# Audio-WestlakeU/FN-SSL

Hardware: AMD Instinct MI355X
Metric: TF-frames/sec DP-IPD forward, 4-mic 257-bin x 300-frame (higher is better)
Workload: dtype f32; 1 GPU; BASELINE configs[1]: FN-SSL (online) DP-IPD forward, waveform->STFT->features->3x(full-band BiLSTM + narrow-band LSTM)->head; 32 utterances/GPU x 4 mics ('MM' = 6 pairs) x 257 bins x 300 frames, fp32; frame = one STFT frame of one utterance; stream_chunk_frames=0, utterances_per_gpu=32, global_batch=32, mics=4, pairs_per_utterance=6, frames=300, bins=257, parallelism=dp1 (utterance shards, no collective), chunk_pairs=0

## Files before the change

fn-ssl_amd/csrc/lstm_f32c.h:

```cpp
#pragma once

#include "lstm_static.h"

namespace fnssl_lstm {

constexpr int kF32cWaves = 16;

struct F32ClusterParams {
  unsigned* tags;
  unsigned* status;
  int clusters_per_dir;
  int groups_per_cluster;
  unsigned spin_limit;
  int stall_member;
  int rotate;
  int prio_mode;
};

template <int HH, int NV0, int NS0, int MODE, bool ABLRT = false, int DRIFT = 2, int NW_ = kF32cWaves, int GS = 1>
__global__ void __launch_bounds__(NW_ * 64) lstm_f32c_kernel(const LstmParams p, const F32ClusterParams cp) {
  constexpr int H = HH, NS = H / 16, NW = NW_;
  constexpr int NWS = NW / GS;
  static_assert((GS == 1 || GS == 4) && NW % GS == 0 && (NWS & (NWS - 1)) == 0, "gate split: whole slots, a power of two of them");
  constexpr bool SUM = (MODE & kSum) != 0, SAVE = (MODE & kSave) != 0;
  constexpr bool CAT = (MODE & kHas2) != 0;
  constexpr int QPS = 1 + NV0 + NS0 + NS;
  constexpr int XD = NW_ > 12 ? 4 : 8;
  constexpr bool STRH = H == 256 && GS == 1 && NW_ > 8;
  static_assert((CAT ? NS0 == 1 : !(NV0 && NS0)) && (NV0 == 0 || NV0 % XD == 0) && (H == 128 || H == 256),
                "blocks of src0, or its remainder alone, or blocks of src0 + the remainder quad of src2");
  static_assert(H == 128 || NW_ <= 8 || STRH, "H = 256 with the row of h_{t-1} held: at most two waves per SIMD (register budget)");
  static_assert(!STRH || (NV0 >= XD && (NV0 + NS) % XD == 0), "streamed row: the ring depth divides the block count");
  static_assert(GS == 1 || (!SAVE && !ABLRT), "gate split: inference kernels only");
  extern __shared__ __attribute__((aligned(16))) char smem[];
  const int ABL = ABLRT ? p.ablate : 0;

  const int b = blockIdx.x;
  const int m = (b >> 3) % NS;
  const int cl = ((b >> 3) / NS) * 8 + (b & 7);
  if (cl >= cp.clusters_per_dir * p.ndir) return;
  const int dir = cl / cp.clusters_per_dir;
  const int ck = cl - dir * cp.clusters_per_dir;
  const int g0 = ck * cp.groups_per_cluster;
  const int g1 = g0 + cp.groups_per_cluster < p.ntasks ? g0 + cp.groups_per_cluster : p.ntasks;
  if (__hip_atomic_load(cp.status, __ATOMIC_RELAXED, __HIP_MEMORY_SCOPE_AGENT) != 0) return;
  if (cl == 0 && m == cp.stall_member) return;

  const int lane = threadIdx.x & 63;
  const int n = lane & 15, g = lane >> 4;
  const int w = __builtin_amdgcn_readfirstlane((int)(threadIdx.x >> 6));
  const int ws = GS == 1 ? w : (w >> 2);
  const int gate = GS == 1 ? 0 : (w & 3);
  const bool rev = dir == 1;
  const unsigned vlane = lane * 16;

  {
    const v4f* src = reinterpret_cast<const v4f*>(reinterpret_cast<const char*>(p.wpack[dir]) + (size_t)(m * QPS) * 4096);
    v4f* dst = reinterpret_cast<v4f*>(smem);
    for (int i = threadIdx.x; i < QPS * 4 * 64; i += NW * 64) dst[i] = src[i];
  }
  char* const xch = smem + QPS * 4096;
  unsigned* const xcnt = reinterpret_cast<unsigned*>(xch + NWS * 2 * 4 * 1024);
  if (GS > 1 && threadIdx.x < NWS) xcnt[threadIdx.x] = 0;
  __syncthreads();
  const char* const lds_rd = smem + lane * 16;
  auto rec = [&](int q, int j) { return *reinterpret_cast<const v4f*>(lds_rd + (q * 4 + j) * 1024); };
  auto rec1 = [&](int q, int j) { return *reinterpret_cast<const float*>(lds_rd + (q * 4 + j) * 1024 + 4 * gate); };

  const unsigned st0 = (unsigned)(p.src0.st * 4), sto = (unsigned)(p.out_st * 4), stk = SUM ? (unsigned)(p.skip.st * 4) : 0u;
  const unsigned st2 = CAT ? (unsigned)(p.src2.st * 4) : 0u;
  const unsigned cy = (unsigned)p.carry;
  unsigned* const tag_cl = cp.tags + (size_t)cl * cp.groups_per_cluster * NS;
  const v4f zero4 = v4f{0.f, 0.f, 0.f, 0.f};

  unsigned pub_val = 0;
  unsigned* pub_tag = nullptr;
  auto pub_flush = [&]() {
    if (pub_tag) {
      asm volatile("s_waitcnt vmcnt(0)" ::: "memory");
      if (lane == 0) __hip_atomic_store(pub_tag, pub_val, __ATOMIC_RELAXED, __HIP_MEMORY_SCOPE_AGENT);
      pub_tag = nullptr;
    }
  };

  struct Grp {
    unsigned vo0, voo, vok, voo2, vo2 = 0;
    bool valid;
    int task, step;
  };
  auto locate = [&](int task, int qo0, int qi0, Grp& gr, rsrc_t& rx0, rsrc_t& ro, rsrc_t& rsk, rsrc_t& ro2, rsrc_t& rx2) {
    const int q0 = task * 16;
    gr.valid = q0 + n < p.nseq;
    const int d = q0 + n < p.nseq ? n : p.nseq - 1 - q0;
    const bool crossed = qi0 + d >= p.q_inner;
    auto one = [&](const float* base, long long so, long long si, int extra, unsigned& voff) {
      const long long delta = (long long)d * si + (crossed ? so - (long long)p.q_inner * si : 0ll);
      voff = (unsigned)(delta * 4) + (unsigned)(extra * 4);
      return make_rsrc(base + ((long long)qo0 * so + (long long)qi0 * si));
    };
    rx0 = one(p.src0.p, p.src0.so, p.src0.si, (NS0 && !CAT) ? g : 4 * g, gr.vo0);
    if constexpr (CAT) rx2 = one(p.src2.p, p.src2.so, p.src2.si, g, gr.vo2);
    ro = one(p.out, p.out_so, p.out_si, dir * H + 4 * g, gr.voo);
    gr.vok = gr.voo2 = 0;
    rsk = SUM ? one(p.skip.p, p.skip.so, p.skip.si, dir * H + 4 * g, gr.vok) : rx0;
    ro2 = SUM ? one(p.out_sum, p.out_so, p.out_si, dir * H + 4 * g, gr.voo2) : ro;
  };
  auto tt_of = [&](int step) { return (unsigned)(rev ? p.nsteps - 1 - step : step); };
  auto rc_of = [&](int task) {
    return make_rsrc(cell_record<NS>(p.cscratch, p.ntasks, dir, task));
  };

  if (g0 + ws >= g1) return;
  unsigned long long clk0 = 0, rt0 = 0;
  if (ABLRT && (ABL & 512)) {
    clk0 = __builtin_amdgcn_s_memtime();
    rt0 = __builtin_amdgcn_s_memrealtime();
  }
  bool dead = false;
  auto bounded_wait = [&](auto ready, auto reload, int sleep, unsigned code) {
    for (unsigned spins = 0; !ready(); ++spins) {
      if (GS > 1) __builtin_amdgcn_s_sleep(1); else if (sleep == 8) __builtin_amdgcn_s_sleep(8); else __builtin_amdgcn_s_sleep(16);
      reload();
      const bool out = spins > cp.spin_limit;
      if (out || (spins & 63) == 63) {
        if (out) {
          if (lane == 0) __hip_atomic_store(cp.status, code | (unsigned)(cl & 0xffff), __ATOMIC_RELAXED, __HIP_MEMORY_SCOPE_AGENT);
          return false;
        }
        if (__hip_atomic_load(cp.status, __ATOMIC_RELAXED, __HIP_MEMORY_SCOPE_AGENT) != 0) return false;
      }
    }
    return true;
  };
  const int NGR = g1 - g0;
  const bool rot = cp.rotate && NGR >= 2 * NWS;
  const int FULL = rot ? (NGR / NWS) * NWS : NGR, LEFT = NGR - FULL;
  const bool single = GS == 1 && g0 + ws + NWS >= g1;
  Grp cur, nxt;
  rsrc_t rx0, ro, rsk, ro2, rx2, nrx0, nro, nrsk, nro2, nrx2;
  v4f xr[XD];
  float xs0 = 0.f;
  v4f cprev = zero4, skipv = zero4;
  unsigned tagv = 0, tagd = 0;
  auto request = [&](const Grp& gr, rsrc_t qx0, rsrc_t qsk, bool with_c, bool with_x = true) {
    const unsigned tt = tt_of(gr.step);
    if (!(ABL & 8)) {
      if constexpr (NV0 > 0) if (with_x) static_for<XD>([&](auto v) { xr[v.value] = bld4(qx0, gr.vo0, tt * st0 + 64 * v.value); });
      if constexpr (NS0 > 0 && !CAT) xs0 = bld1(qx0, gr.vo0, tt * st0);
    }
    if (SUM && !(ABL & 64)) skipv = bld4(qsk, gr.vok, tt * stk + 64 * m);
    if (gr.step > 0 || cy) {
      if (gr.step > 0 && !(ABL & 256))
        tagv = __hip_atomic_load(tag_cl + (size_t)(gr.task - g0) * NS + (lane & (NS - 1)), __ATOMIC_RELAXED, __HIP_MEMORY_SCOPE_AGENT);
      if (GS == 1 && with_c && !(ABL & 64)) cprev = bld4_l2(rc_of(gr.task), vlane, m * 1024);
    }
    if (DRIFT > 0 && !(ABL & 256) && gr.task - DRIFT * NWS >= g0)
      tagd = __hip_atomic_load(tag_cl + (size_t)(gr.task - DRIFT * NWS - g0) * NS + (lane & (NS - 1)), __ATOMIC_RELAXED, __HIP_MEMORY_SCOPE_AGENT);
  };
  cur.task = g0 + ws;
  cur.step = 0;
  unsigned iter = 0;
  const int qo_first = (cur.task * 16) / p.q_inner, qi_first = cur.task * 16 - qo_first * p.q_inner;
  int qo0 = qo_first, qi0 = qi_first;
  locate(cur.task, qo0, qi0, cur, rx0, ro, rsk, ro2, rx2);
  request(cur, rx0, rsk, true);
  if constexpr (CAT) xs0 = bld1(rx2, cur.vo2, tt_of(0) * st2);

  for (;;) {
    const int step = cur.step, task = cur.task;
    const unsigned tt = tt_of(step);
    const unsigned o0 = tt * st0, oo = (tt + cy) * sto;
    const unsigned op = (rev ? tt + 1 : tt - 1 + cy) * sto;
    const rsrc_t rc = rc_of(task);
    unsigned* const tag_g = tag_cl + (size_t)(task - g0) * NS;
    if (single && (step > 0 || cy) && !(ABL & 64)) cprev = bld4_l2(rc, vlane, m * 1024);
    const bool late_c = GS > 1 || task >= g0 + FULL;
    v4f cprev_cur = (step > 0 || cy) ? cprev : zero4;
    const v4f skip_cur = skipv;

    v4f hold[STRH ? 1 : NS];
    auto fetch_h = [&]() {
      if (DRIFT > 0 && !(ABL & 4) && !dead && task - DRIFT * NWS >= g0) {
        unsigned* const tag_d = tag_cl + (size_t)(task - DRIFT * NWS - g0) * NS;
        dead = !bounded_wait([&]() { return __builtin_amdgcn_ballot_w64(tagd < (unsigned)step + 1) == 0; },
                             [&]() { tagd = __hip_atomic_load(tag_d + (lane & (NS - 1)), __ATOMIC_RELAXED, __HIP_MEMORY_SCOPE_AGENT); }, 8, 0x40000u);
      }
      if ((step > 0 || cy) && !(ABL & 16)) {
        if (step > 0 && !(ABL & 4) && !dead)
          dead = !bounded_wait([&]() { return __builtin_amdgcn_ballot_w64(tagv < (unsigned)step) == 0; },
                               [&]() { tagv = __hip_atomic_load(tag_g + (lane & (NS - 1)), __ATOMIC_RELAXED, __HIP_MEMORY_SCOPE_AGENT); }, 16, 0x30000u);
        if (late_c && !(ABL & 64)) cprev_cur = bld4_l2(rc, vlane, m * 1024);
        if constexpr (!STRH) {
#pragma unroll
          for (int s = 0; s < NS; ++s) hold[s] = bld4_l2(ro, cur.voo, op + 64 * s);
        }
      } else if constexpr (!STRH) {
#pragma unroll
        for (int s = 0; s < NS; ++s) hold[s] = (ABL & 16) ? cprev : zero4;
      }
    };
    const bool hrow = step > 0 || cy;
    auto hblock = [&](int j) { return hrow ? bld4_l2(ro, cur.voo, op + 64 * j) : zero4; };

    if (cp.prio_mode == 2) __builtin_amdgcn_s_setprio(2);
    v4f acc[4];
    v4f ra[4];
    v4f acc1 = zero4;
    float rb[4] = {0.f, 0.f, 0.f, 0.f};
    if constexpr (GS == 1) {
      acc[0] = rec(0, 0);
      acc[1] = rec(0, 1);
      acc[2] = rec(0, 2);
      acc[3] = rec(0, 3);
      static_for<4>([&](auto j) { ra[j.value] = rec(1, j.value); });
    } else {
      acc1 = rec(0, gate);
      static_for<4>([&](auto j) { rb[j.value] = rec1(1, j.value); });
    }
    auto quad = [&](auto qc, float b0, float b1, float b2, float b3) {
      constexpr int Q = decltype(qc)::value;
      if constexpr (GS > 1) {
        acc1 = __builtin_amdgcn_mfma_f32_16x16x4f32(rb[0], b0, acc1, 0, 0, 0);
        if constexpr (Q + 1 < QPS) rb[0] = rec1(Q + 1, 0);
        acc1 = __builtin_amdgcn_mfma_f32_16x16x4f32(rb[1], b1, acc1, 0, 0, 0);
        if constexpr (Q + 1 < QPS) rb[1] = rec1(Q + 1, 1);
        acc1 = __builtin_amdgcn_mfma_f32_16x16x4f32(rb[2], b2, acc1, 0, 0, 0);
        if constexpr (Q + 1 < QPS) rb[2] = rec1(Q + 1, 2);
        acc1 = __builtin_amdgcn_mfma_f32_16x16x4f32(rb[3], b3, acc1, 0, 0, 0);
        if constexpr (Q + 1 < QPS) rb[3] = rec1(Q + 1, 3);
        return;
      }
      MFMA4(acc, ra[0], b0);
      __builtin_amdgcn_sched_barrier(0);
      if constexpr (Q + 1 < QPS) if (!(ABL & 128)) ra[0] = rec(Q + 1, 0);
      __builtin_amdgcn_sched_barrier(0);
      MFMA4(acc, ra[1], b1);
      __builtin_amdgcn_sched_barrier(0);
      if constexpr (Q + 1 < QPS) if (!(ABL & 128)) ra[1] = rec(Q + 1, 1);
      __builtin_amdgcn_sched_barrier(0);
      MFMA4(acc, ra[2], b2);
      __builtin_amdgcn_sched_barrier(0);
      if constexpr (Q + 1 < QPS) if (!(ABL & 128)) ra[2] = rec(Q + 1, 2);
      __builtin_amdgcn_sched_barrier(0);
      MFMA4(acc, ra[3], b3);
      __builtin_amdgcn_sched_barrier(0);
      if constexpr (Q + 1 < QPS) if (!(ABL & 128)) ra[3] = rec(Q + 1, 3);
      __builtin_amdgcn_sched_barrier(0);
    };
    auto quad1 = [&](auto qc, float b0) {
      constexpr int Q = decltype(qc)::value;
      if constexpr (GS > 1) {
        acc1 = __builtin_amdgcn_mfma_f32_16x16x4f32(rb[0], b0, acc1, 0, 0, 0);
        if constexpr (Q + 1 < QPS) static_for<4>([&](auto j) { rb[j.value] = rec1(Q + 1, j.value); });
        return;
      }
      MFMA4(acc, ra[0], b0);
      if constexpr (Q + 1 < QPS) static_for<4>([&](auto j) { ra[j.value] = rec(Q + 1, j.value); });
    };
    if constexpr (NV0 > 0) {
      static_for<NV0>([&](auto v) {
        constexpr int V = decltype(v)::value;
        if constexpr (STRH) {
          if constexpr (V == NV0 / 2) pub_flush();
          if constexpr (V == NV0 - XD) fetch_h();
        } else if constexpr (V == NV0 / 2) {
          pub_flush();
          fetch_h();
        }
        const v4f xb = xr[V % XD];
        quad(ic<1 + V>{}, xb.x, xb.y, xb.z, xb.w);
        if constexpr (V + XD < NV0) {
          if (!(ABL & 8)) xr[V % XD] = bld4(rx0, cur.vo0, o0 + 64 * (V + XD));
        } else if constexpr (STRH) {
          xr[V % XD] = hblock(V + XD - NV0);
        }
      });
      if constexpr (NS0 > 0) quad1(ic<1 + NV0>{}, xs0);
    } else {
      pub_flush();
      fetch_h();
      quad1(ic<1>{}, xs0);
    }
    bool seq_next = false;
    if (task < g0 + FULL && task + NWS < g0 + FULL) {
      nxt.task = task + NWS;
      nxt.step = step;
      seq_next = true;
    } else {
      const int j = (ws - step) & (NWS - 1);
      if (task < g0 + FULL && j < LEFT) {
        nxt.task = g0 + FULL + j;
        nxt.step = step;
      } else {
        nxt.task = g0 + ws;
        nxt.step = step + 1;
      }
    }
    const bool more = nxt.step < p.nsteps;
    if (more) {
      if (ABL & 1) {
        nxt.vo0 = cur.vo0; nxt.voo = cur.voo; nxt.vok = cur.vok; nxt.voo2 = cur.voo2; nxt.valid = cur.valid;
        nrx0 = rx0; nro = ro; nrsk = rsk; nro2 = ro2;
        if constexpr (CAT) {
          nxt.vo2 = cur.vo2;
          nrx2 = rx2;
        }
      } else {
        if (seq_next) {
          qi0 += 16 * NWS;
          while (qi0 >= p.q_inner) {
            qi0 -= p.q_inner;
            ++qo0;
          }
        } else if (nxt.step == step) {
          qo0 = (nxt.task * 16) / p.q_inner;
          qi0 = nxt.task * 16 - qo0 * p.q_inner;
        } else {
          qo0 = qo_first;
          qi0 = qi_first;
        }
        locate(nxt.task, qo0, qi0, nxt, nrx0, nro, nrsk, nro2, nrx2);
      }
      request(nxt, nrx0, nrsk, !single && nxt.task < g0 + FULL, !STRH);
      if constexpr (CAT) xs0 = bld1(nrx2, nxt.vo2, tt_of(nxt.step) * st2);
    }
    static_for<NS>([&](auto sp) {
      constexpr int SP = decltype(sp)::value;
      if constexpr (STRH) {
        constexpr int B = NV0 + SP, B2 = B + XD;
        const v4f hb = xr[B % XD];
        quad(ic<1 + NV0 + NS0 + SP>{}, hb.x, hb.y, hb.z, hb.w);
        if constexpr (B2 < NV0 + NS) {
          xr[B % XD] = hblock(B2 - NV0);
        } else {
          if (more) xr[B % XD] = bld4(nrx0, nxt.vo0, tt_of(nxt.step) * st0 + 64 * (B2 - NV0 - NS));
        }
      } else {
        quad(ic<1 + NV0 + NS0 + SP>{}, hold[SP].x, hold[SP].y, hold[SP].z, hold[SP].w);
      }
    });

    if (cp.prio_mode == 2) __builtin_amdgcn_s_setprio(0);
    if (dead) break;
    v4f cn, hn;
    if (ABL & 2) {
      cn = acc[1] + cprev_cur + acc[0];
      hn = acc[3] + acc[2];
    } else {
      v4f ig, fg, gg, og;
      if constexpr (GS == 1) {
        ig = sigmoid4(acc[0]);
        fg = sigmoid4(acc[1]);
        gg = tanh4(acc[2]);
        og = sigmoid4(acc[3]);
      } else {
        const v4f act = gate == 2 ? tanh4(acc1) : sigmoid4(acc1);
        v4f* const xb = reinterpret_cast<v4f*>(xch + (size_t)((ws * 2 + (int)(iter & 1u)) * 4) * 1024);
        xb[gate * 64 + lane] = act;
        asm volatile("s_waitcnt lgkmcnt(0)" ::: "memory");
        if (lane == 0) __hip_atomic_fetch_add(xcnt + ws, 1u, __ATOMIC_RELAXED, __HIP_MEMORY_SCOPE_WORKGROUP);
        const unsigned want = 4u * (iter + 1u);
        for (unsigned spins = 0;; ++spins) {
          if (__hip_atomic_load(xcnt + ws, __ATOMIC_RELAXED, __HIP_MEMORY_SCOPE_WORKGROUP) >= want) break;
          if (dead || ((spins & 63u) == 63u && __hip_atomic_load(cp.status, __ATOMIC_RELAXED, __HIP_MEMORY_SCOPE_AGENT) != 0u) ||
              spins > cp.spin_limit) {
            dead = true;
            break;
          }
          __builtin_amdgcn_s_sleep(1);
        }
        asm volatile("" ::: "memory");
        ig = xb[lane];
        fg = xb[64 + lane];
        gg = xb[128 + lane];
        og = xb[192 + lane];
        ++iter;
      }
      cn = cell4(fg, cprev_cur, ig, gg);
      hn = mul_rn4(og, tanh4(cn));
      if constexpr (SAVE) {
        const rsrc_t rres = make_rsrc(reinterpret_cast<const char*>(p.reserve) +
                                      ((size_t)dir * p.ntasks + task) * p.nsteps * (size_t)(NS * kReserveRecs * 1024));
        const unsigned rb = (tt * NS + m) * (kReserveRecs * 1024);
        bst4(ig, rres, vlane, rb);
        bst4(fg, rres, vlane, rb + 1024);
        bst4(gg, rres, vlane, rb + 2048);
        bst4(og, rres, vlane, rb + 3072);
        bst4(cn, rres, vlane, rb + 4096);
      }
    }
    asm("" : "+v"(hn.x), "+v"(hn.y), "+v"(hn.z), "+v"(hn.w));
    if (ABL & 32) asm volatile("" ::"v"(cn), "v"(hn));
    const bool storer = GS == 1 || gate == 0;
    if (storer && !(ABL & 32)) bst4(cn, rc, vlane, m * 1024);
    if (storer && cur.valid && !(ABL & 32)) {
      __builtin_amdgcn_raw_buffer_store_b128(__builtin_bit_cast(v4u, hn), ro, cur.voo, oo + 64 * m, 16);
      if (SUM) bst4(add_rn4(hn, skip_cur), ro2, cur.voo2, oo + 64 * m);
    }
    pub_val = __builtin_amdgcn_readfirstlane((unsigned)step + 1);
    pub_tag = ((ABL & 256) || !storer) ? nullptr : tag_g + m;
    if (GS > 1 || single) pub_flush();
    if (!more || dead) break;
    cur = nxt;
    rx0 = nrx0;
    ro = nro;
    rsk = nrsk;
    ro2 = nro2;
    if constexpr (CAT) rx2 = nrx2;
  }
  pub_flush();
  asm volatile("s_waitcnt vmcnt(0)" ::: "memory");
  if (ABLRT && (ABL & 512) && (w == 0 || w == 15) && lane == 0) {
    const unsigned long long c1 = __builtin_amdgcn_s_memtime(), r1 = __builtin_amdgcn_s_memrealtime();
    printf("f32c blk %d wave %d start %llu end %llu cycles %llu MHz %.1f\n", b, w, rt0, r1, c1 - clk0,
           (double)(c1 - clk0) / (double)(r1 - rt0) * 100.0);
  }
}

template <int HH, int NV0, int NS0, int MODE, bool ABLRT = false, int DRIFT = 2, int NW_ = kF32cWaves, int GS = 1>
int launch_f32c_k(const LstmParams& p, const F32ClusterParams& cp, const LaunchCtx& lc) {
  constexpr int NS = HH / 16;
  constexpr int QPS = 1 + NV0 + NS0 + NS;
  const size_t lds = (size_t)QPS * 4096 + (GS > 1 ? (size_t)(NW_ / GS) * 8192 + 64 : 0);
  static_assert(QPS * 4096 + (GS > 1 ? (NW_ / GS) * 8192 + 64 : 0) <= 160 * 1024, "LDS");
  const int ncl = cp.clusters_per_dir * p.ndir;
  const int nwg = 8 * NS * ((ncl + 7) / 8);
  return enqueue(lc, Kernel{lstm_f32c_kernel<HH, NV0, NS0, MODE, ABLRT, DRIFT, NW_, GS>, NW_ * 64, lds, "lstm_f32c_kernel", true}, nwg, p, cp);
}

}
```

fn-ssl_amd/csrc/lstm_f32c.hip:

```cpp
#include <cstdlib>

#include "lstm_f32c.h"
#include "tuning.h"

namespace fnssl_lstm {

constexpr int kF32cWavesH256 = 16;
constexpr int kF32cWavesH256Split = 8;

static bool f32c_uniform(const LstmParams& p, int mode) {
  auto even = [&](long long so, long long si) { return si >= 0 && so == (long long)p.q_inner * si; };
  return even(p.src0.so, p.src0.si) && even(p.out_so, p.out_si) && (!(mode & kSum) || even(p.skip.so, p.skip.si)) &&
         (!(mode & kHas2) || even(p.src2.so, p.src2.si));
}

bool f32c_handles(const LstmParams& p, int H, int mode) {
  if (fnssl::tune(FNSSL_TUNE_NO_F32_CLUSTER)) return false;
  if ((H != 128 && H != 256) || p.ablate) return false;
  if (H == 128) {
    if (p.c2 != 0 || p.carry) return false;
    if (p.reserve && mode != 0) return false;
    if (!(p.c0 == 256 && (mode == kSum || mode == 0)) && !(p.c0 == 4 && mode == 0 && !fnssl::tune(FNSSL_TUNE_NO_F32C_B1))) return false;
  } else {
    if (p.ndir != 1 || p.c0 != 256 || fnssl::tune(FNSSL_TUNE_NO_F32_SMALL)) return false;
    const bool plain = p.c2 == 0 && (mode == 0 || mode == kSum), cat = p.c2 == 4 && (mode == kHas2 || mode == (kHas2 | kSum));
    if (!plain && !cat) return false;
    if (p.reserve && ((mode & kSum) || p.carry)) return false;
  }
  auto grows = [&](long long so, long long si) { return si >= 0 && so >= (long long)(p.q_inner - 1) * si; };
  if (!f32c_uniform(p, mode) &&
      (p.q_inner < 16 || !grows(p.src0.so, p.src0.si) || !grows(p.out_so, p.out_si) ||
       ((mode & kSum) && !grows(p.skip.so, p.skip.si)) || ((mode & kHas2) && !grows(p.src2.so, p.src2.si))))
    return false;
  const int ncu = cluster_cus();
  if (ncu < (H / 16) * p.ndir) return false;
  const long long groups = (long long)p.ntasks * p.ndir;
  if (const int mg = fnssl::tune(FNSSL_TUNE_F32C_MIN_GROUPS, 1, 1 << 30)) {
    if (groups < mg) return false;
  }
  if (p.reserve) {
    if (fnssl::tune(FNSSL_TUNE_TRAIN_NO_F32_CLUSTER)) return false;
    return true;
  }
  if (H == 256) {
    const long long full = 12LL * ncu, rounds = (groups + full - 1) / full;
    return groups < full || groups * 100 < rounds * full * 97;
  }
  return !fnssl::tune(FNSSL_TUNE_NO_F32_SMALL) || groups >= 12LL * ncu;
}

template <int NW_, int GS>
static int launch_f32c_h256(const LstmParams& p, const F32ClusterParams& cp, int mode, const LaunchCtx& lc) {
  if (mode == (kHas2 | kSum)) return launch_f32c_k<256, 16, 1, kHas2 | kSum, false, 2, NW_, GS>(p, cp, lc);
  if (mode == kHas2) return launch_f32c_k<256, 16, 1, kHas2, false, 2, NW_, GS>(p, cp, lc);
  if (mode == kSum) return launch_f32c_k<256, 16, 0, kSum, false, 2, NW_, GS>(p, cp, lc);
  return launch_f32c_k<256, 16, 0, 0, false, 2, NW_, GS>(p, cp, lc);
}

int forward_f32c(LstmParams p, int H, int mode, size_t cluster_bytes, const LaunchCtx& lc) {
  if (f32c_uniform(p, mode)) p.q_inner = p.nseq;
  const int ncu = cluster_cus();
  const int members = H / 16;
  F32ClusterParams cp;
  cp.clusters_per_dir = (ncu / members) / p.ndir;
  cp.groups_per_cluster = (p.ntasks + cp.clusters_per_dir - 1) / cp.clusters_per_dir;
  cp.status = reinterpret_cast<unsigned*>(p.cluster_ws);
  cp.tags = reinterpret_cast<unsigned*>(p.cluster_ws + 256);
  cp.spin_limit = cluster_spin_limit();
  cp.stall_member = cluster_test_stall();
  cp.rotate = !fnssl::tune(FNSSL_TUNE_F32C_NO_ROTATE);
  cp.prio_mode = fnssl::tune(FNSSL_TUNE_F32C_PRIO, 9, 9) ? 0 : 2;
  const size_t tag_bytes = (size_t)p.ndir * cp.clusters_per_dir * cp.groups_per_cluster * members * sizeof(unsigned);
  FNSSL_REQUIRE(256 + tag_bytes <= cluster_bytes, "lstm_forward: the cluster kernel's tags exceed the workspace's cluster area");
  if (!lc.dry) FNSSL_HIP(hipMemsetAsync(p.cluster_ws, 0, 256 + tag_bytes, lc.st));
  const int gs_knob = fnssl::tune(FNSSL_TUNE_F32C_GATE_SPLIT, 1, 4);
  const bool gsplit = gs_knob ? gs_knob == 4 : cp.groups_per_cluster <= 1;
  if (H == 256) {
    constexpr int W = kF32cWavesH256;
    if (p.reserve)
      return p.c2 == 4 ? launch_f32c_k<256, 16, 1, kHas2 | kSave, false, 2, W>(p, cp, lc) : launch_f32c_k<256, 16, 0, kSave, false, 2, W>(p, cp, lc);
    if (gsplit) return launch_f32c_h256<kF32cWavesH256Split, 4>(p, cp, mode, lc);
    if (cp.groups_per_cluster <= kF32cWavesH256Split) return launch_f32c_h256<kF32cWavesH256Split, 1>(p, cp, mode, lc);
    return launch_f32c_h256<W, 1>(p, cp, mode, lc);
  }
  if (gsplit && !p.reserve) {
    if (p.c0 == 4) return launch_f32c_k<128, 0, 1, 0, false, 2, kF32cWaves, 4>(p, cp, lc);
    if (mode == kSum) return launch_f32c_k<128, 16, 0, kSum, false, 2, kF32cWaves, 4>(p, cp, lc);
    return launch_f32c_k<128, 16, 0, 0, false, 2, kF32cWaves, 4>(p, cp, lc);
  }
#ifdef FNSSL_BUILD_ABLATE
  if (const int abl = env_int("FNSSL_F32C_ABL", 1, 1023)) {
    p.ablate = abl;
    if (mode == kSum) return launch_f32c_k<128, 16, 0, kSum, true>(p, cp, lc);
    if (p.c0 == 4) return launch_f32c_k<128, 0, 1, 0, true>(p, cp, lc);
  }
  p.ablate = 0;
#endif
  if (p.reserve) return p.c0 == 4 ? launch_f32c_k<128, 0, 1, kSave>(p, cp, lc) : launch_f32c_k<128, 16, 0, kSave>(p, cp, lc);
  if (p.c0 == 4) return launch_f32c_k<128, 0, 1, 0>(p, cp, lc);
  if (mode == kSum) return launch_f32c_k<128, 16, 0, kSum>(p, cp, lc);
  return launch_f32c_k<128, 16, 0, 0>(p, cp, lc);
}

}
```

Measured before the change: 17990 frames/s.

## Precompute per-group buffer offsets in an LDS table and keep one resource per tensor

```diff
diff --git a/fn-ssl_amd/csrc/lstm_f32c.h b/fn-ssl_amd/csrc/lstm_f32c.h
--- a/fn-ssl_amd/csrc/lstm_f32c.h
+++ b/fn-ssl_amd/csrc/lstm_f32c.h
@@ -5,6 +5,16 @@
 namespace fnssl_lstm {
 
 constexpr int kF32cWaves = 16;
+
+constexpr int kF32cEntryWords = 5;
+constexpr size_t kF32cLaneTableBytes = 64 * 16;
+constexpr size_t kF32cLdsLimit = 160 * 1024;
+__host__ __device__ constexpr size_t f32c_lane_table_offset(int qps, int slots) {
+  return (size_t)qps * 4096 + (slots ? (size_t)slots * 8192 + 64 : 0);
+}
+__host__ __device__ constexpr size_t f32c_lds_bytes(int qps, int slots, int groups_per_cluster) {
+  return f32c_lane_table_offset(qps, slots) + kF32cLaneTableBytes + (((size_t)groups_per_cluster * kF32cEntryWords * 4 + 15) & ~(size_t)15);
+}
 
 struct F32ClusterParams {
   unsigned* tags;
@@ -62,10 +72,44 @@
   char* const xch = smem + QPS * 4096;
   unsigned* const xcnt = reinterpret_cast<unsigned*>(xch + NWS * 2 * 4 * 1024);
   if (GS > 1 && threadIdx.x < NWS) xcnt[threadIdx.x] = 0;
+  constexpr int LT = (int)f32c_lane_table_offset(QPS, GS > 1 ? NWS : 0);
+  unsigned* const gtab = reinterpret_cast<unsigned*>(smem + LT + kF32cLaneTableBytes);
+  const int qob = (g0 * 16) / p.q_inner, qib = g0 * 16 - qob * p.q_inner;
+  for (int t = threadIdx.x; t < g1 - g0; t += NW * 64) {
+    const int q0 = (g0 + t) * 16;
+    const int qo = q0 / p.q_inner, qi = q0 - qo * p.q_inner;
+    auto off = [&](long long so, long long si) { return (unsigned)(((long long)(qo - qob) * so + (long long)(qi - qib) * si) * 4); };
+    unsigned* const e = gtab + t * kF32cEntryWords;
+    e[0] = off(p.src0.so, p.src0.si);
+    e[1] = CAT ? off(p.src2.so, p.src2.si) : 0u;
+    e[2] = off(p.out_so, p.out_si);
+    e[3] = SUM ? off(p.skip.so, p.skip.si) : 0u;
+    const int xl = p.q_inner - qi < 16 ? p.q_inner - qi : 16;
+    const int live = p.nseq - q0 < 16 ? p.nseq - q0 : 16;
+    e[4] = (unsigned)xl | ((unsigned)live << 8);
+  }
+  if (w == 0) {
+    auto ln = [&](long long si, int extra) { return (unsigned)n * (unsigned)(si * 4) + (unsigned)(extra * 4); };
+    unsigned* const e = reinterpret_cast<unsigned*>(smem + LT) + lane * 4;
+    e[0] = ln(p.src0.si, (NS0 && !CAT) ? g : 4 * g);
+    e[1] = CAT ? ln(p.src2.si, g) : 0u;
+    e[2] = ln(p.out_si, dir * H + 4 * g);
+    e[3] = SUM ? ln(p.skip.si, dir * H + 4 * g) : 0u;
+  }
   __syncthreads();
   const char* const lds_rd = smem + lane * 16;
-  auto rec = [&](int q, int j) { return *reinterpret_cast<const v4f*>(lds_rd + (q * 4 + j) * 1024); };
-  auto rec1 = [&](int q, int j) { return *reinterpret_cast<const float*>(lds_rd + (q * 4 + j) * 1024 + 4 * gate); };
+  typedef __attribute__((address_space(3))) const char lds_cc;
+  constexpr int NB = (QPS * 4096 + 65535) / 65536;
+  lds_cc* lds_b[NB];
+  lds_b[0] = (lds_cc*)lds_rd;
+#pragma unroll
+  for (int k = 1; k < NB; ++k) {
+    lds_b[k] = lds_b[0] + k * 65536;
+    asm volatile("" : "+v"(lds_b[k]));
+  }
+  auto rec_at = [&](int q, int j) { return lds_b[((q * 4 + j) * 1024) >> 16] + (((q * 4 + j) * 1024) & 65535); };
+  auto rec = [&](int q, int j) { return *reinterpret_cast<__attribute__((address_space(3))) const v4f*>(rec_at(q, j)); };
+  auto rec1 = [&](int q, int j) { return *reinterpret_cast<__attribute__((address_space(3))) const float*>(rec_at(q, j) + 4 * gate); };
 
   const unsigned st0 = (unsigned)(p.src0.st * 4), sto = (unsigned)(p.out_st * 4), stk = SUM ? (unsigned)(p.skip.st * 4) : 0u;
   const unsigned st2 = CAT ? (unsigned)(p.src2.st * 4) : 0u;
@@ -84,31 +128,48 @@
   };
 
   struct Grp {
-    unsigned vo0, voo, vok, voo2, vo2 = 0;
-    bool valid;
     int task, step;
-  };
-  auto locate = [&](int task, int qo0, int qi0, Grp& gr, rsrc_t& rx0, rsrc_t& ro, rsrc_t& rsk, rsrc_t& ro2, rsrc_t& rx2) {
-    const int q0 = task * 16;
-    gr.valid = q0 + n < p.nseq;
-    const int d = q0 + n < p.nseq ? n : p.nseq - 1 - q0;
-    const bool crossed = qi0 + d >= p.q_inner;
-    auto one = [&](const float* base, long long so, long long si, int extra, unsigned& voff) {
-      const long long delta = (long long)d * si + (crossed ? so - (long long)p.q_inner * si : 0ll);
-      voff = (unsigned)(delta * 4) + (unsigned)(extra * 4);
-      return make_rsrc(base + ((long long)qo0 * so + (long long)qi0 * si));
-    };
-    rx0 = one(p.src0.p, p.src0.so, p.src0.si, (NS0 && !CAT) ? g : 4 * g, gr.vo0);
-    if constexpr (CAT) rx2 = one(p.src2.p, p.src2.so, p.src2.si, g, gr.vo2);
-    ro = one(p.out, p.out_so, p.out_si, dir * H + 4 * g, gr.voo);
-    gr.vok = gr.voo2 = 0;
-    rsk = SUM ? one(p.skip.p, p.skip.so, p.skip.si, dir * H + 4 * g, gr.vok) : rx0;
-    ro2 = SUM ? one(p.out_sum, p.out_so, p.out_si, dir * H + 4 * g, gr.voo2) : ro;
+    unsigned xl;
+  };
+  struct Tensor {
+    rsrc_t r;
+    unsigned si4, xc;
+  };
+  auto tensor = [&](const float* base, long long so, long long si) {
+    Tensor t;
+    t.r = make_rsrc(base + ((long long)qob * so + (long long)qib * si));
+    t.si4 = (unsigned)(si * 4);
+    t.xc = (unsigned)((so - (long long)p.q_inner * si) * 4);
+    return t;
+  };
+  const Tensor T0 = tensor(p.src0.p, p.src0.so, p.src0.si);
+  const Tensor T2 = CAT ? tensor(p.src2.p, p.src2.so, p.src2.si) : T0;
+  const Tensor TO = tensor(p.out, p.out_so, p.out_si);
+  const Tensor TK = SUM ? tensor(p.skip.p, p.skip.so, p.skip.si) : T0;
+  typedef __attribute__((address_space(3))) const unsigned lds_cu;
+  auto lane_part = [&](int W) {
+    lds_cu* q = (lds_cu*)reinterpret_cast<const unsigned*>(lds_rd + LT);
+    asm volatile("" : "+v"(q));
+    return q[W];
+  };
+  const rsrc_t rx0 = T0.r, rx2 = T2.r, ro = TO.r, rsk = TK.r;
+  const rsrc_t ro2 = SUM ? make_rsrc(p.out_sum + ((long long)qob * p.out_so + (long long)qib * p.out_si)) : ro;
+  const rsrc_t rc = make_rsrc(cell_record<NS>(p.cscratch, p.ntasks, dir, g0));
+  auto coff = [&](int task) { return (unsigned)((task - g0) * NS + m) * 1024u; };
+  auto entry = [&](int task) { return gtab + ((ABL & 1) ? ws : task - g0) * kF32cEntryWords; };
+  auto open = [&](Grp& gr) { gr.xl = __builtin_amdgcn_readfirstlane(entry(gr.task)[4]); };
+  auto voff_of = [&](const Grp& gr, int W, const Tensor& t) {
+    const unsigned go = entry(gr.task)[W];
+    const unsigned xlane = gr.xl & 255u, live = gr.xl >> 8;
+    const unsigned ln = lane_part(W);
+    unsigned v = go + ln + ((unsigned)n >= xlane ? t.xc : 0u);
+    if (__builtin_expect(live < 16u, 0)) {
+      const unsigned last = go + ln - ((unsigned)n - (live - 1u)) * t.si4 + (live - 1u >= xlane ? t.xc : 0u);
+      if ((unsigned)n >= live) v = last;
+    }
+    return v;
   };
   auto tt_of = [&](int step) { return (unsigned)(rev ? p.nsteps - 1 - step : step); };
-  auto rc_of = [&](int task) {
-    return make_rsrc(cell_record<NS>(p.cscratch, p.ntasks, dir, task));
-  };
 
   if (g0 + ws >= g1) return;
   unsigned long long clk0 = 0, rt0 = 0;
@@ -137,22 +198,24 @@
   const int FULL = rot ? (NGR / NWS) * NWS : NGR, LEFT = NGR - FULL;
   const bool single = GS == 1 && g0 + ws + NWS >= g1;
   Grp cur, nxt;
-  rsrc_t rx0, ro, rsk, ro2, rx2, nrx0, nro, nrsk, nro2, nrx2;
+  unsigned vo0 = 0, voo;
   v4f xr[XD];
   float xs0 = 0.f;
   v4f cprev = zero4, skipv = zero4;
   unsigned tagv = 0, tagd = 0;
-  auto request = [&](const Grp& gr, rsrc_t qx0, rsrc_t qsk, bool with_c, bool with_x = true) {
+  auto request = [&](const Grp& gr, bool with_c, bool with_x = true) {
     const unsigned tt = tt_of(gr.step);
+    if constexpr (NV0 > 0 || (NS0 > 0 && !CAT)) vo0 = voff_of(gr, 0, T0);
     if (!(ABL & 8)) {
-      if constexpr (NV0 > 0) if (with_x) static_for<XD>([&](auto v) { xr[v.value] = bld4(qx0, gr.vo0, tt * st0 + 64 * v.value); });
-      if constexpr (NS0 > 0 && !CAT) xs0 = bld1(qx0, gr.vo0, tt * st0);
-    }
-    if (SUM && !(ABL & 64)) skipv = bld4(qsk, gr.vok, tt * stk + 64 * m);
+      if constexpr (NV0 > 0) if (with_x) static_for<XD>([&](auto v) { xr[v.value] = bld4(rx0, vo0, tt * st0 + 64 * v.value); });
+      if constexpr (NS0 > 0 && !CAT) xs0 = bld1(rx0, vo0, tt * st0);
+    }
+    if constexpr (CAT) xs0 = bld1(rx2, voff_of(gr, 1, T2), tt * st2);
+    if (SUM && !(ABL & 64)) skipv = bld4(rsk, voff_of(gr, 3, TK), tt * stk + 64 * m);
     if (gr.step > 0 || cy) {
       if (gr.step > 0 && !(ABL & 256))
         tagv = __hip_atomic_load(tag_cl + (size_t)(gr.task - g0) * NS + (lane & (NS - 1)), __ATOMIC_RELAXED, __HIP_MEMORY_SCOPE_AGENT);
-      if (GS == 1 && with_c && !(ABL & 64)) cprev = bld4_l2(rc_of(gr.task), vlane, m * 1024);
+      if (GS == 1 && with_c && !(ABL & 64)) cprev = bld4_l2(rc, vlane, coff(gr.task));
     }
     if (DRIFT > 0 && !(ABL & 256) && gr.task - DRIFT * NWS >= g0)
       tagd = __hip_atomic_load(tag_cl + (size_t)(gr.task - DRIFT * NWS - g0) * NS + (lane & (NS - 1)), __ATOMIC_RELAXED, __HIP_MEMORY_SCOPE_AGENT);
@@ -160,20 +223,18 @@
   cur.task = g0 + ws;
   cur.step = 0;
   unsigned iter = 0;
-  const int qo_first = (cur.task * 16) / p.q_inner, qi_first = cur.task * 16 - qo_first * p.q_inner;
-  int qo0 = qo_first, qi0 = qi_first;
-  locate(cur.task, qo0, qi0, cur, rx0, ro, rsk, ro2, rx2);
-  request(cur, rx0, rsk, true);
-  if constexpr (CAT) xs0 = bld1(rx2, cur.vo2, tt_of(0) * st2);
+  open(cur);
+  request(cur, true);
+  voo = voff_of(cur, 2, TO);
 
   for (;;) {
     const int step = cur.step, task = cur.task;
     const unsigned tt = tt_of(step);
     const unsigned o0 = tt * st0, oo = (tt + cy) * sto;
     const unsigned op = (rev ? tt + 1 : tt - 1 + cy) * sto;
-    const rsrc_t rc = rc_of(task);
+    const unsigned oc = coff(task);
     unsigned* const tag_g = tag_cl + (size_t)(task - g0) * NS;
-    if (single && (step > 0 || cy) && !(ABL & 64)) cprev = bld4_l2(rc, vlane, m * 1024);
+    if (single && (step > 0 || cy) && !(ABL & 64)) cprev = bld4_l2(rc, vlane, oc);
     const bool late_c = GS > 1 || task >= g0 + FULL;
     v4f cprev_cur = (step > 0 || cy) ? cprev : zero4;
     const v4f skip_cur = skipv;
@@ -189,10 +250,10 @@
         if (step > 0 && !(ABL & 4) && !dead)
           dead = !bounded_wait([&]() { return __builtin_amdgcn_ballot_w64(tagv < (unsigned)step) == 0; },
                                [&]() { tagv = __hip_atomic_load(tag_g + (lane & (NS - 1)), __ATOMIC_RELAXED, __HIP_MEMORY_SCOPE_AGENT); }, 16, 0x30000u);
-        if (late_c && !(ABL & 64)) cprev_cur = bld4_l2(rc, vlane, m * 1024);
+        if (late_c && !(ABL & 64)) cprev_cur = bld4_l2(rc, vlane, oc);
         if constexpr (!STRH) {
 #pragma unroll
-          for (int s = 0; s < NS; ++s) hold[s] = bld4_l2(ro, cur.voo, op + 64 * s);
+          for (int s = 0; s < NS; ++s) hold[s] = bld4_l2(ro, voo, op + 64 * s);
         }
       } else if constexpr (!STRH) {
 #pragma unroll
@@ -200,7 +261,7 @@
       }
     };
     const bool hrow = step > 0 || cy;
-    auto hblock = [&](int j) { return hrow ? bld4_l2(ro, cur.voo, op + 64 * j) : zero4; };
+    auto hblock = [&](int j) { return hrow ? bld4_l2(ro, voo, op + 64 * j) : zero4; };
 
     if (cp.prio_mode == 2) __builtin_amdgcn_s_setprio(2);
     v4f acc[4];
@@ -270,7 +331,7 @@
         const v4f xb = xr[V % XD];
         quad(ic<1 + V>{}, xb.x, xb.y, xb.z, xb.w);
         if constexpr (V + XD < NV0) {
-          if (!(ABL & 8)) xr[V % XD] = bld4(rx0, cur.vo0, o0 + 64 * (V + XD));
+          if (!(ABL & 8)) xr[V % XD] = bld4(rx0, vo0, o0 + 64 * (V + XD));
         } else if constexpr (STRH) {
           xr[V % XD] = hblock(V + XD - NV0);
         }
@@ -281,11 +342,9 @@
       fetch_h();
       quad1(ic<1>{}, xs0);
     }
-    bool seq_next = false;
     if (task < g0 + FULL && task + NWS < g0 + FULL) {
       nxt.task = task + NWS;
       nxt.step = step;
-      seq_next = true;
     } else {
       const int j = (ws - step) & (NWS - 1);
       if (task < g0 + FULL && j < LEFT) {
@@ -298,31 +357,8 @@
     }
     const bool more = nxt.step < p.nsteps;
     if (more) {
-      if (ABL & 1) {
-        nxt.vo0 = cur.vo0; nxt.voo = cur.voo; nxt.vok = cur.vok; nxt.voo2 = cur.voo2; nxt.valid = cur.valid;
-        nrx0 = rx0; nro = ro; nrsk = rsk; nro2 = ro2;
-        if constexpr (CAT) {
-          nxt.vo2 = cur.vo2;
-          nrx2 = rx2;
-        }
-      } else {
-        if (seq_next) {
-          qi0 += 16 * NWS;
-          while (qi0 >= p.q_inner) {
-            qi0 -= p.q_inner;
-            ++qo0;
-          }
-        } else if (nxt.step == step) {
-          qo0 = (nxt.task * 16) / p.q_inner;
-          qi0 = nxt.task * 16 - qo0 * p.q_inner;
-        } else {
-          qo0 = qo_first;
-          qi0 = qi_first;
-        }
-        locate(nxt.task, qo0, qi0, nxt, nrx0, nro, nrsk, nro2, nrx2);
-      }
-      request(nxt, nrx0, nrsk, !single && nxt.task < g0 + FULL, !STRH);
-      if constexpr (CAT) xs0 = bld1(nrx2, nxt.vo2, tt_of(nxt.step) * st2);
+      open(nxt);
+      request(nxt, !single && nxt.task < g0 + FULL, !STRH);
     }
     static_for<NS>([&](auto sp) {
       constexpr int SP = decltype(sp)::value;
@@ -333,7 +369,7 @@
         if constexpr (B2 < NV0 + NS) {
           xr[B % XD] = hblock(B2 - NV0);
         } else {
-          if (more) xr[B % XD] = bld4(nrx0, nxt.vo0, tt_of(nxt.step) * st0 + 64 * (B2 - NV0 - NS));
+          if (more) xr[B % XD] = bld4(rx0, vo0, tt_of(nxt.step) * st0 + 64 * (B2 - NV0 - NS));
         }
       } else {
         quad(ic<1 + NV0 + NS0 + SP>{}, hold[SP].x, hold[SP].y, hold[SP].z, hold[SP].w);
@@ -392,21 +428,17 @@
     asm("" : "+v"(hn.x), "+v"(hn.y), "+v"(hn.z), "+v"(hn.w));
     if (ABL & 32) asm volatile("" ::"v"(cn), "v"(hn));
     const bool storer = GS == 1 || gate == 0;
-    if (storer && !(ABL & 32)) bst4(cn, rc, vlane, m * 1024);
-    if (storer && cur.valid && !(ABL & 32)) {
-      __builtin_amdgcn_raw_buffer_store_b128(__builtin_bit_cast(v4u, hn), ro, cur.voo, oo + 64 * m, 16);
-      if (SUM) bst4(add_rn4(hn, skip_cur), ro2, cur.voo2, oo + 64 * m);
+    if (storer && !(ABL & 32)) bst4(cn, rc, vlane, oc);
+    if (storer && (unsigned)n < (cur.xl >> 8) && !(ABL & 32)) {
+      __builtin_amdgcn_raw_buffer_store_b128(__builtin_bit_cast(v4u, hn), ro, voo, oo + 64 * m, 16);
+      if (SUM) bst4(add_rn4(hn, skip_cur), ro2, voo, oo + 64 * m);
     }
     pub_val = __builtin_amdgcn_readfirstlane((unsigned)step + 1);
     pub_tag = ((ABL & 256) || !storer) ? nullptr : tag_g + m;
     if (GS > 1 || single) pub_flush();
     if (!more || dead) break;
     cur = nxt;
-    rx0 = nrx0;
-    ro = nro;
-    rsk = nrsk;
-    ro2 = nro2;
-    if constexpr (CAT) rx2 = nrx2;
+    voo = voff_of(cur, 2, TO);
   }
   pub_flush();
   asm volatile("s_waitcnt vmcnt(0)" ::: "memory");
@@ -421,8 +453,9 @@
 int launch_f32c_k(const LstmParams& p, const F32ClusterParams& cp, const LaunchCtx& lc) {
   constexpr int NS = HH / 16;
   constexpr int QPS = 1 + NV0 + NS0 + NS;
-  const size_t lds = (size_t)QPS * 4096 + (GS > 1 ? (size_t)(NW_ / GS) * 8192 + 64 : 0);
-  static_assert(QPS * 4096 + (GS > 1 ? (NW_ / GS) * 8192 + 64 : 0) <= 160 * 1024, "LDS");
+  const size_t lds = f32c_lds_bytes(QPS, GS > 1 ? NW_ / GS : 0, cp.groups_per_cluster);
+  static_assert(f32c_lds_bytes(QPS, GS > 1 ? NW_ / GS : 0, 1) <= kF32cLdsLimit, "LDS");
+  FNSSL_REQUIRE(lds <= kF32cLdsLimit, "lstm_forward: the cluster kernel's group table (%d groups per cluster) exceeds the LDS", cp.groups_per_cluster);
   const int ncl = cp.clusters_per_dir * p.ndir;
   const int nwg = 8 * NS * ((ncl + 7) / 8);
   return enqueue(lc, Kernel{lstm_f32c_kernel<HH, NV0, NS0, MODE, ABLRT, DRIFT, NW_, GS>, NW_ * 64, lds, "lstm_f32c_kernel", true}, nwg, p, cp);
diff --git a/fn-ssl_amd/csrc/lstm_f32c.hip b/fn-ssl_amd/csrc/lstm_f32c.hip
--- a/fn-ssl_amd/csrc/lstm_f32c.hip
+++ b/fn-ssl_amd/csrc/lstm_f32c.hip
@@ -1,3 +1,4 @@
+#include <algorithm>
 #include <cstdlib>
 
 #include "lstm_f32c.h"
@@ -12,6 +13,39 @@
   auto even = [&](long long so, long long si) { return si >= 0 && so == (long long)p.q_inner * si; };
   return even(p.src0.so, p.src0.si) && even(p.out_so, p.out_si) && (!(mode & kSum) || even(p.skip.so, p.skip.si)) &&
          (!(mode & kHas2) || even(p.src2.so, p.src2.si));
+}
+
+struct F32cGeometry {
+  int clusters_per_dir, groups_per_cluster;
+  bool gate_split;
+};
+static F32cGeometry f32c_geometry(const LstmParams& p, int H) {
+  F32cGeometry ge;
+  ge.clusters_per_dir = (cluster_cus() / (H / 16)) / p.ndir;
+  ge.groups_per_cluster = (p.ntasks + ge.clusters_per_dir - 1) / ge.clusters_per_dir;
+  const int gs_knob = fnssl::tune(FNSSL_TUNE_F32C_GATE_SPLIT, 1, 4);
+  ge.gate_split = !p.reserve && (gs_knob ? gs_knob == 4 : ge.groups_per_cluster <= 1);
+  return ge;
+}
+
+static bool f32c_table_applies(LstmParams p, int H, int mode) {
+  if (f32c_uniform(p, mode)) p.q_inner = p.nseq;
+  const F32cGeometry ge = f32c_geometry(p, H);
+  const int slots = ge.gate_split ? (H == 256 ? 8 : kF32cWaves) / 4 : 0;
+  if (f32c_lds_bytes(p.quads_per_slice, slots, ge.groups_per_cluster) > kF32cLdsLimit) return false;
+  auto span_ok = [&](long long so, long long si, long long st) {
+    auto at = [&](long long q) { return (long double)(q / p.q_inner) * so + (long double)(q % p.q_inner) * si; };
+    for (int ck = 0; ck < ge.clusters_per_dir; ++ck) {
+      const long long qa = (long long)ck * ge.groups_per_cluster * 16;
+      if (qa >= p.nseq) break;
+      const long long qz = std::min<long long>(qa + (long long)ge.groups_per_cluster * 16, p.nseq) - 1;
+      const long double bytes = ((at(qz) - at(qa)) + (long double)(p.nsteps + p.carry) * st + 2 * H) * 4;
+      if (bytes >= 4294967296.0L) return false;
+    }
+    return true;
+  };
+  return span_ok(p.src0.so, p.src0.si, p.src0.st) && span_ok(p.out_so, p.out_si, p.out_st) &&
+         (!(mode & kSum) || span_ok(p.skip.so, p.skip.si, p.skip.st)) && (!(mode & kHas2) || span_ok(p.src2.so, p.src2.si, p.src2.st));
 }
 
 bool f32c_handles(const LstmParams& p, int H, int mode) {
@@ -34,6 +68,7 @@
     return false;
   const int ncu = cluster_cus();
   if (ncu < (H / 16) * p.ndir) return false;
+  if (!f32c_table_applies(p, H, mode)) return false;
   const long long groups = (long long)p.ntasks * p.ndir;
   if (const int mg = fnssl::tune(FNSSL_TUNE_F32C_MIN_GROUPS, 1, 1 << 30)) {
     if (groups < mg) return false;
@@ -59,11 +94,11 @@
 
 int forward_f32c(LstmParams p, int H, int mode, size_t cluster_bytes, const LaunchCtx& lc) {
   if (f32c_uniform(p, mode)) p.q_inner = p.nseq;
-  const int ncu = cluster_cus();
   const int members = H / 16;
+  const F32cGeometry ge = f32c_geometry(p, H);
   F32ClusterParams cp;
-  cp.clusters_per_dir = (ncu / members) / p.ndir;
-  cp.groups_per_cluster = (p.ntasks + cp.clusters_per_dir - 1) / cp.clusters_per_dir;
+  cp.clusters_per_dir = ge.clusters_per_dir;
+  cp.groups_per_cluster = ge.groups_per_cluster;
   cp.status = reinterpret_cast<unsigned*>(p.cluster_ws);
   cp.tags = reinterpret_cast<unsigned*>(p.cluster_ws + 256);
   cp.spin_limit = cluster_spin_limit();
@@ -73,8 +108,7 @@
   const size_t tag_bytes = (size_t)p.ndir * cp.clusters_per_dir * cp.groups_per_cluster * members * sizeof(unsigned);
   FNSSL_REQUIRE(256 + tag_bytes <= cluster_bytes, "lstm_forward: the cluster kernel's tags exceed the workspace's cluster area");
   if (!lc.dry) FNSSL_HIP(hipMemsetAsync(p.cluster_ws, 0, 256 + tag_bytes, lc.st));
-  const int gs_knob = fnssl::tune(FNSSL_TUNE_F32C_GATE_SPLIT, 1, 4);
-  const bool gsplit = gs_knob ? gs_knob == 4 : cp.groups_per_cluster <= 1;
+  const bool gsplit = ge.gate_split;
   if (H == 256) {
     constexpr int W = kF32cWavesH256;
     if (p.reserve)
@@ -83,7 +117,7 @@
     if (cp.groups_per_cluster <= kF32cWavesH256Split) return launch_f32c_h256<kF32cWavesH256Split, 1>(p, cp, mode, lc);
     return launch_f32c_h256<W, 1>(p, cp, mode, lc);
   }
-  if (gsplit && !p.reserve) {
+  if (gsplit) {
     if (p.c0 == 4) return launch_f32c_k<128, 0, 1, 0, false, 2, kF32cWaves, 4>(p, cp, lc);
     if (mode == kSum) return launch_f32c_k<128, 16, 0, kSum, false, 2, kF32cWaves, 4>(p, cp, lc);
     return launch_f32c_k<128, 16, 0, 0, false, 2, kF32cWaves, 4>(p, cp, lc);
```

Result: no change. 18100 frames/s (median of 6 runs) (+0.7%).
